# John-Jumper/Upside-MD

Hardware: AMD Instinct MI355X
Metric: MD steps/sec (force evals/sec) per 300-res protein (higher is better)
Workload: dtype f32; 1 GPU; syn300_10A: 300-res synthetic protein, full side-chain BP, 10 A pair list (BASELINE.json configs[2]); 4096 independent replicas per GPU, T=0.8, dt=0.009, Langevin thermostat every round; replicas_per_gpu=4096, n_atom=900, settle_steps=100

## Files before the change

upside-md_amd/csrc/engine.cpp:

```cpp
#include "engine.h"
#include "h5util.h"
#include <dlfcn.h>
#include <algorithm>
#include <cstdlib>
#include <set>
#include <functional>
#include <cmath>
#include <cstdio>
#include <cstring>

using namespace std;

void hip_check(hipError_t e, const char* what) {
    if (e != hipSuccess) throw string("HIP error in ") + what + ": " + hipGetErrorString(e);
}
void upk_check(int code, const char* what) {
    if (code == 0) return;
    if (code >= 9000) {
        const char* why = "";
        switch (code) {
            case 9003: why = ": more than 1024 rotamer nodes"; break;
            case 9004: case 9005: case 9006: why = ": the system does not fit the 160 KB of LDS this kernel stages it in"; break;
            case 9007: case 9008: why = ": side / mode / interaction type outside what the launcher implements"; break;
            case 9009: why = ": more than 65535 rows (row ids are 16 bits wide)"; break;
            case 9010: why = ": the graph's pair lists were allocated with another word width than its kernels read (upk_igraph_t::word16: 16-bit element "
                             "indices for every graph but the rotamer's, <= 65534 elements per side)"; break;
            case 9011: why = ": the hit-list refine exists for the side-chain graph (symmetric, 32-bit words) and for two-sided graphs with 16-bit words; "
                             "a symmetric radial graph walks its cached lists and has no hit lists"; break;
            default: break;
        }
        throw string("kernel launcher ") + what + " rejected its arguments (code " + to_string(code) + ")" + why;
    }
    throw string("HIP launch failure in ") + what + ": " + hipGetErrorString((hipError_t)code);
}

void DeviceCtx::flush() { upk_check(upk_fuse_flush(&L), "fuse_flush"); }
void DeviceCtx::begin(const std::string& fam) {
    if (!profile) return;
    flush();
    hipEvent_t a, b;
    hip_check(hipEventCreate(&a), "hipEventCreate"); hip_check(hipEventCreate(&b), "hipEventCreate");
    hip_check(hipEventRecord(a, stream), "hipEventRecord");
    families[fam].pending.emplace_back(a, b);
}
void DeviceCtx::end(const std::string& fam, double algorithmic_bytes, double pair_evaluations) {
    if (!profile) return;
    flush();
    auto& f = families[fam];
    hip_check(hipEventRecord(f.pending.back().second, stream), "hipEventRecord");
    f.launches += 1; f.bytes += algorithmic_bytes; f.pairs += pair_evaluations;
}
void DeviceCtx::flush_profile() {
    for (auto& kv : families) {
        for (auto& ev : kv.second.pending) {
            hip_check(hipEventSynchronize(ev.second), "hipEventSynchronize");
            float ms = 0.f;
            hip_check(hipEventElapsedTime(&ms, ev.first, ev.second), "hipEventElapsedTime");
            kv.second.ms += ms;
            (void)hipEventDestroy(ev.first); (void)hipEventDestroy(ev.second);
        }
        kv.second.pending.clear();
    }
}

int ScatterPlan::add_source(int n_term, int n_slot, int w, const vector<int>& targets) {
    if (finalized) throw string("scatter plan already finalized");
    if ((int)targets.size() != n_term * n_slot) throw string("scatter source: wrong target table size");
    if (width && width != w) throw string("scatter sources of one node must share a width");
    width = w;
    Source s; s.n_term = n_term; s.n_slot = n_slot; s.width = w; s.targets = targets; s.offset = arena_size;
    arena_size += (long)n_term * n_slot * w;
    sources.push_back(move(s));
    return (int)sources.size() - 1;
}
void ScatterPlan::finalize(int n_target, int n_system) {
    vector<int> count(n_target + 1, 0);
    for (auto& s : sources) for (int t : s.targets) if (t >= 0) { if (t >= n_target) throw string("scatter target out of range"); count[t + 1]++; }
    for (int t = 0; t < n_target; ++t) count[t + 1] += count[t];
    vector<int> fill(count.begin(), count.end() - 1), entry(count[n_target]);
    for (auto& s : sources)
        for (int i = 0; i < (int)s.targets.size(); ++i) {
            int t = s.targets[i];
            if (t >= 0) entry[fill[t]++] = (int)(s.offset + (long)i * s.width);
        }
    csr_start.upload(count); csr_entry.upload(entry);
    arena.alloc((size_t)n_system * (size_t)max(arena_size, 1L));
    finalized = true;
}

CoordNode::CoordNode(DeviceCtx* c, int n_elem_, int elem_width_)
    : DerivComputation(false), n_elem(n_elem_), elem_width(elem_width_), stride(ru(elem_width_)) {
    ctx = c;
    output.alloc((size_t)c->n_system * n_elem * stride);
    sens.alloc((size_t)c->n_system * n_elem * stride);
}
void CoordNode::gather_contributions() {
    if (scatter.sources.empty()) return;
    upk_check(upk_gather_contrib(&ctx->L, scatter.arena.p, scatter.arena_size, scatter.csr_start.p, scatter.csr_entry.p, coord(),
                                 scatter.width, 0), "gather_contrib");
}

namespace {
vector<int> identity_targets(int n) { vector<int> v(n); for (int i = 0; i < n; ++i) v[i] = i; return v; }

void fetch_dense(DeviceCtx* ctx, const CoordNode& n, const float* dev, vector<float>& stage, vector<float>& dst) {
    const size_t total = (size_t)ctx->n_system * n.n_elem * n.stride;
    stage.resize(total); dst.resize((size_t)ctx->n_system * n.n_elem * n.elem_width);
    if (!total) return;
    hip_check(hipMemcpyAsync(stage.data(), dev, total * sizeof(float), hipMemcpyDeviceToHost, ctx->stream), "D2H");
    hip_check(hipStreamSynchronize(ctx->stream), "hipStreamSynchronize");
    for (size_t e = 0; e < (size_t)ctx->n_system * n.n_elem; ++e)
        for (int d = 0; d < n.elem_width; ++d) dst[e * n.elem_width + d] = stage[e * n.stride + d];
}

void push_arg_derivs(DeviceCtx* ctx, const vector<CoordNode*>& args, const vector<int>& src, const vector<vector<float>>& din) {
    for (size_t a = 0; a < args.size(); ++a) {
        CoordNode& n = *args[a];
        const size_t per_sys = (size_t)n.n_elem * n.elem_width;
        for (int s = 0; s < ctx->n_system && per_sys; ++s)
            hip_check(hipMemcpyAsync(n.scatter.source_ptr(src[a]) + (size_t)s * n.scatter.arena_size, din[a].data() + s * per_sys,
                                     per_sys * sizeof(float), hipMemcpyHostToDevice, ctx->stream), "H2D");
    }
    hip_check(hipStreamSynchronize(ctx->stream), "hipStreamSynchronize");
}
}

HostPotentialNode::HostPotentialNode(DeviceCtx* c, const vector<CoordNode*>& args_) : PotentialNode(c), args(args_) {
    for (CoordNode* a : args) src_.push_back(a->scatter.add_source(a->n_elem, 1, a->elem_width, identity_targets(a->n_elem)));
    in_.resize(args.size()); din_.resize(args.size()); stage_.resize(args.size());
}
void HostPotentialNode::compute_value(ComputeMode) {
    for (size_t a = 0; a < args.size(); ++a) {
        fetch_dense(ctx, *args[a], args[a]->output.p, stage_[a], in_[a]);
        din_[a].assign(in_[a].size(), 0.f);
    }
    vector<const float*> in(args.size()); vector<float*> din(args.size());
    for (int s = 0; s < ctx->n_system; ++s) {
        for (size_t a = 0; a < args.size(); ++a) {
            const size_t off = (size_t)s * args[a]->n_elem * args[a]->elem_width;
            in[a] = in_[a].data() + off; din[a] = din_[a].data() + off;
        }
        potential[s] = host_potential(s, in, din);
    }
    hip_check(hipMemcpyAsync(potential_dev.p, potential.data(), ctx->n_system * sizeof(float), hipMemcpyHostToDevice, ctx->stream), "H2D");
    push_arg_derivs(ctx, args, src_, din_);
}

HostCoordNode::HostCoordNode(DeviceCtx* c, int n_elem_, int elem_width_, const vector<CoordNode*>& args_)
    : CoordNode(c, n_elem_, elem_width_), args(args_) {
    for (CoordNode* a : args) src_.push_back(a->scatter.add_source(a->n_elem, 1, a->elem_width, identity_targets(a->n_elem)));
    in_.resize(args.size()); din_.resize(args.size()); stage_.resize(args.size());
}
void HostCoordNode::compute_value(ComputeMode) {
    for (size_t a = 0; a < args.size(); ++a) fetch_dense(ctx, *args[a], args[a]->output.p, stage_[a], in_[a]);
    out_.assign((size_t)ctx->n_system * n_elem * stride, 0.f);
    vector<const float*> in(args.size()); vector<float> dense((size_t)n_elem * elem_width);
    for (int s = 0; s < ctx->n_system; ++s) {
        for (size_t a = 0; a < args.size(); ++a) in[a] = in_[a].data() + (size_t)s * args[a]->n_elem * args[a]->elem_width;
        host_value(s, in, dense.data());
        for (int e = 0; e < n_elem; ++e) for (int d = 0; d < elem_width; ++d) out_[((size_t)s * n_elem + e) * stride + d] = dense[(size_t)e * elem_width + d];
    }
    if (!out_.empty()) hip_check(hipMemcpyAsync(output.p, out_.data(), out_.size() * sizeof(float), hipMemcpyHostToDevice, ctx->stream), "H2D");
    hip_check(hipStreamSynchronize(ctx->stream), "hipStreamSynchronize");
}
void HostCoordNode::propagate_deriv() {
    vector<float> stage;
    fetch_dense(ctx, *this, sens.p, stage, dout_);
    vector<const float*> in(args.size()); vector<float*> din(args.size());
    for (size_t a = 0; a < args.size(); ++a) din_[a].assign(in_[a].size(), 0.f);
    for (int s = 0; s < ctx->n_system; ++s) {
        for (size_t a = 0; a < args.size(); ++a) {
            const size_t off = (size_t)s * args[a]->n_elem * args[a]->elem_width;
            in[a] = in_[a].data() + off; din[a] = din_[a].data() + off;
        }
        host_deriv(s, in, dout_.data() + (size_t)s * n_elem * elem_width, din);
    }
    push_arg_derivs(ctx, args, src_, din_);
}

NodeCreationMap& node_creation_map() {
    static NodeCreationMap m;
// ... 892 lines not shown
```

upside-md_amd/csrc/kernels_igraph.hip:

```cpp
#include "igraph_device.h"
#include <cstring>

using namespace up;

#define ST(L) ((hipStream_t)(L)->stream)
#define ROWS_PER_BLOCK 4
#define IG_BLOCK (ROWS_PER_BLOCK * UP_WAVE)
#ifndef UPK_LAUNCH_STATUS_DEFINED
#define UPK_LAUNCH_STATUS_DEFINED
static inline int launch_status() { return (int)hipGetLastError(); }
#endif
static inline unsigned rows_grid(int n_rows) { return n_rows > 0 ? (unsigned)((n_rows + ROWS_PER_BLOCK - 1) / ROWS_PER_BLOCK) : 1u; }

#define C_OUT(c, s)  ((c).out  + (size_t)(s) * (c).n_elem * (c).stride)
#define C_SENS(c, s) ((c).sens + (size_t)(s) * (c).n_elem * (c).stride)


__device__ __forceinline__ float quadspline(const upk_igraph_t& G, const float* __restrict__ p, const float* x1, const float* x2,
                                            float* d1, float* d2) {
    const int ka = G.n_knot_angular, k = G.n_knot;
    const float inv_dx = G.inv_dx, inv_dtheta = G.inv_dtheta;
    const f3 displace = mk3(x2[0] - x1[0], x2[1] - x1[1], x2[2] - x1[2]);
    const f3 rvec1 = mk3(x1[3], x1[4], x1[5]), rvec2 = mk3(x2[3], x2[4], x2[5]);
    const float dist2 = mag2(displace), inv_dist = rsqrt_(dist2);
// ... 113 lines not shown
    }
    __syncthreads();
    if (moved) {
        for (int e = threadIdx.x; e < n_tot; e += blockDim.x) {
            const bool side1 = e < G.n1;
            const int i = side1 ? e : e - G.n1;
            const upk_coord_t& node = side1 ? G.node1 : G.node2;
            const float* x = C_OUT(node, s) + (size_t)(side1 ? G.loc1[i] : G.loc2[i]) * node.stride;
            float4* c = (float4*)(side1 ? G.cache_pos1 + (size_t)s * G.n1 * 4 : G.cache_pos2 + (size_t)s * G.n2 * 4) + i;
            *c = make_float4(x[0], x[1], x[2], __int_as_float(side1 ? G.id1[i] : G.id2[i]));
        }
        if (G.mark_table) {
            uint4* m = (uint4*)(G.mark_table + (size_t)s * G.mark_stride);
            const int n16 = G.mark_stride / 16;
            for (int i = threadIdx.x; i < n16; i += blockDim.x) m[i] = make_uint4(0, 0, 0, 0);
        }
    }
    if (threadIdx.x == 0) {
        G.rebuild_flag[s] = moved;
        int* fl = UPK_FLAG_LIST(G);
        if (moved) fl[1 + atomicAdd(&fl[0], 1)] = s;
        if (s == 0) G.flagged[(size_t)(G.parity ^ 1) * G.flag_stride] = 0;
    }
}
__global__ void k_pairlist_check(upk_igraph_t G)  { d_pairlist_check(G, BX_REAL, nullptr); }
extern "C" int upk_pairlist_check(const upk_launch_t* L, const upk_igraph_t* G) {
    if (batch_add(L, BK_CHECK, 1, L->n_system, 0, G, sizeof(*G))) return 0;
    UPK_FLUSH(L);
    const int n_tot = G->symmetric ? G->n1 : G->n1 + G->n2;
    const int threads = plan_upkeep_block(L->n_system, upk_device_cu_count(), n_tot <= 256 ? 256 : (n_tot <= 512 ? 512 : 1024));
    hipLaunchKernelGGL(k_pairlist_check, dim3(1, L->n_system), dim3(threads), 0, ST(L), *G);
    return launch_status();
}

template <int IT>
__device__ __forceinline__ bool plb_id_ok(int id_row_side1, int id_other_side2) {
    if (IT == UPK_IT_ROTAMER) return ((unsigned)(id_row_side1 ^ id_other_side2)) > 15u;
    if (IT == UPK_IT_HBOND_COVERAGE || IT == UPK_IT_ENVIRONMENT || IT == UPK_IT_RADIAL || IT == UPK_IT_HBOND_SC_RADIAL) { const int d = id_row_side1 - id_other_side2; return (d > 2) | (d < -2); }
    return true;
}
__device__ __forceinline__ int plb_node_of(const upk_igraph_t& G, int id) {
    const int nr = (id >> 4) & 15;
    return (id >> 8) + ((-(int)(nr == 6) & G.mark_start6) | (-(int)(nr == 3) & G.mark_start3));
}
template <bool STAGED, int IT>
__device__ __forceinline__ void d_pairlist_build(const upk_igraph_t& G, int blocks1, int rows_per_wg, const BX B, float* plb_lds) {
        float4* oth = (float4*)plb_lds;
    constexpr bool SYM = IT == UPK_IT_ROTAMER || IT == UPK_IT_RADIAL;
    constexpr bool UPPER = IT == UPK_IT_ROTAMER;
    const int* fl = UPK_FLAG_LIST(G);
    const int n_flagged = fl[0];
    const int lane = threadIdx.x & 63, wave = __builtin_amdgcn_readfirstlane(threadIdx.x >> 6), n_wave = blockDim.x >> 6;
    const bool side1 = (int)B.bx < blocks1;
    const int rb = side1 ? B.bx : B.bx - blocks1;
    const int n_my = side1 ? G.n1 : G.n2, n_other = side1 ? G.n2 : G.n1;
    const int n_pad = (n_other + 63) & ~63;
    const int cap = side1 ? G.cap1 : G.cap2;
    const float cut2 = G.cache_cutoff * G.cache_cutoff;
    for (int fi = B.by; fi < n_flagged; fi += B.gy) {
        const int s = fl[1 + fi];
        const float4* src = (const float4*)((side1 ? G.cache_pos2 : G.cache_pos1) + (size_t)s * n_other * 4);
        const float4* mine = (const float4*)((side1 ? G.cache_pos1 : G.cache_pos2) + (size_t)s * n_my * 4);
        if (STAGED) {
            __syncthreads();
            for (int j = threadIdx.x; j < n_pad; j += blockDim.x) oth[j] = j < n_other ? src[j] : make_float4(1e18f, 1e18f, 1e18f, 0.f);
            __syncthreads();
        }
        float4 x_next = make_float4(0.f, 0.f, 0.f, 0.f);
        { const int i0 = rb * rows_per_wg + wave; if (wave < rows_per_wg && i0 < n_my) x_next = mine[i0]; }
        for (int r = wave; r < rows_per_wg; r += n_wave) {
            const int i = rb * rows_per_wg + r;
            if (i >= n_my) break;
            const float4 x = x_next;
            { const int in = i + n_wave; if (r + n_wave < rows_per_wg && in < n_my) x_next = mine[in]; }
            const int my_id = __float_as_int(x.w);
            typedef typename list_word<IT>::type W;
            W* nbr = (side1 ? (W*)G.nbr1 + (size_t)s * G.n1 * G.cap1 : (W*)G.nbr2 + (size_t)s * G.n2 * G.cap2) + (size_t)i * cap;
            int count = 0;
            const int my_node = SYM ? plb_node_of(G, my_id) : 0;
            for (int j0 = UPPER ? ((i + 1) & ~63) : 0; j0 < n_pad; j0 += 64) {
                const int j = j0 + lane;
                float4 y;
                if (STAGED) y = oth[j];
                else y = j < n_other ? src[j] : make_float4(1e18f, 1e18f, 1e18f, 0.f);
                const float d2 = dist2_exact(x.x, x.y, x.z, y.x, y.y, y.z);
                const int oid = __float_as_int(y.w);
                bool hit = (d2 < cut2) & (side1 ? plb_id_ok<IT>(my_id, oid) : plb_id_ok<IT>(oid, my_id));
                if (UPPER) hit = hit & (j > i);
                else if (SYM) hit = hit & (j != i);
                const unsigned long long b = __ballot(hit);
                if (!b) continue;
                const int pos = count + __popcll(b & ((1ull << lane) - 1ull));
                if (hit & (pos < cap)) nbr[pos] = (W)j;
                count += __popcll(b);
                if (SYM && G.mark_table) {
                    const bool up = hit & (j > i);
                    const int key = up ? plb_node_of(G, oid) : -1;
                    const int key_prev = __builtin_amdgcn_update_dpp(-1, key, 0x138 , 0xf, 0xf, false);
                    if (up & (key_prev != key)) {
                        unsigned char* mt = G.mark_table + (size_t)s * G.mark_stride;
                        mt[my_node * G.mark_ld + key] = 1; mt[key * G.mark_ld + my_node] = 1;
                    }
                }
            }
            if (lane == 0) {
                (side1 ? G.cnt1 + (size_t)s * G.n1 : G.cnt2 + (size_t)s * G.n2)[i] = count < cap ? count : cap;
                if (count > cap) *G.error_flag = 1;
            }
        }
    }
}
template <bool STAGED, int IT>
__global__ void __launch_bounds__(1024) k_pairlist_build(upk_igraph_t G, int blocks1, int rows_per_wg)  {
    extern __shared__ __attribute__((aligned(16))) float lds_dyn_[];
    d_pairlist_build<STAGED, IT>(G, blocks1, rows_per_wg, BX_REAL, lds_dyn_);
}
template <int IT>
static void plb_launch(const upk_launch_t* L, const upk_igraph_t* G, dim3 grid, size_t lds, bool staged, int blocks1) {
    const int rows = plan_list_build_rows(L->n_system, upk_device_cu_count());
    if (staged) hipLaunchKernelGGL((k_pairlist_build<true, IT>), grid, dim3(plan_upkeep_block(L->n_system, upk_device_cu_count(), 1024)), lds, ST(L), *G, blocks1, rows);
    else hipLaunchKernelGGL((k_pairlist_build<false, IT>), grid, dim3(1024), 0, ST(L), *G, blocks1, rows);
}
extern "C" int upk_pairlist_build(const upk_launch_t* L, const upk_igraph_t* G) { return upk_pairlist_build_sides(L, G, 3); }
extern "C" int upk_pairlist_build_sides(const upk_launch_t* L, const upk_igraph_t* G, int sides) {
    if (!list_words_match(G)) return 9010;
    const int rows = plan_list_build_rows(L->n_system, upk_device_cu_count());
    const int blocks1 = (sides & 1) ? (G->n1 + rows - 1) / rows : 0;
    const int blocks2 = (G->symmetric || !(sides & 2)) ? 0 : (G->n2 + rows - 1) / rows;
    if (blocks1 + blocks2 == 0) return 0;
    const int n_max = G->n1 > G->n2 ? G->n1 : G->n2;
    const size_t lds = (size_t)((n_max + 63) & ~63) * 16;
    const dim3 grid(blocks1 + blocks2, UPK_FLAG_GRID(L->n_system));
    const bool staged = plan_list_build_staged(plan_switches(), lds);
    if (staged) {
        const int bk = G->itype == UPK_IT_ROTAMER ? BK_BUILD_ROT : G->itype == UPK_IT_HBOND_COVERAGE ? BK_BUILD_COV : G->itype == UPK_IT_ENVIRONMENT ? BK_BUILD_ENV
                     : G->itype == UPK_IT_PROTEIN_HBOND ? BK_BUILD_HB : 0;
        if (bk && batch_add(L, bk, (int)grid.x, (int)grid.y, lds, G, sizeof(*G), nullptr, 0, blocks1, rows)) return 0;
    }
    UPK_FLUSH(L);
    switch (G->itype) {
        case UPK_IT_ROTAMER: plb_launch<UPK_IT_ROTAMER>(L, G, grid, lds, staged, blocks1); break;
        case UPK_IT_HBOND_COVERAGE: plb_launch<UPK_IT_HBOND_COVERAGE>(L, G, grid, lds, staged, blocks1); break;
        case UPK_IT_ENVIRONMENT: plb_launch<UPK_IT_ENVIRONMENT>(L, G, grid, lds, staged, blocks1); break;
        case UPK_IT_RADIAL: plb_launch<UPK_IT_RADIAL>(L, G, grid, lds, staged, blocks1); break;
        case UPK_IT_HBOND_SC_RADIAL: plb_launch<UPK_IT_HBOND_SC_RADIAL>(L, G, grid, lds, staged, blocks1); break;
        default: plb_launch<UPK_IT_PROTEIN_HBOND>(L, G, grid, lds, staged, blocks1); break;
    }
    return launch_status();
}

#ifndef PLR_BLOCK
#define PLR_BLOCK 256
#endif
#ifndef PLR_DEPTH
#define PLR_DEPTH 2
#endif
static_assert(PLR_ROWS <= 64 * (PLR_BLOCK / 64), "a wavefront of the refine keeps the positions and list lengths of its rows one per lane: at most 64 rows per wavefront");
typedef float plr_v2 __attribute__((ext_vector_type(2)));
__device__ __forceinline__ plr_v2 dist2_exact2(plr_v2 ax, plr_v2 ay, plr_v2 az, plr_v2 bx, plr_v2 by, plr_v2 bz) {
#pragma clang fp contract(off)
    const plr_v2 dx = ax - bx, dy = ay - by, dz = az - bz;
    const plr_v2 xx = dx * dx, yy = dy * dy, zz = dz * dz;
    const plr_v2 s = xx + yy;
    return s + zz;
}
template <bool SYM, typename W>
__device__ __forceinline__ void d_pairlist_refine(const upk_igraph_t& G, int side, int rows_per_wg, const BX B, float* plr_lds) {
        float4* oth = (float4*)plr_lds;
    const int s = B.by;
    const int lane = threadIdx.x & 63, wave = __builtin_amdgcn_readfirstlane(threadIdx.x >> 6), n_wave = blockDim.x >> 6;
    const bool rows1 = side == 1;
    const int n_rows = rows1 ? G.n1 : G.n2, n_other = rows1 ? G.n2 : G.n1;
    const int cap = rows1 ? G.cap1 : G.cap2;
    const float4* src = (const float4*)((rows1 ? G.cur_pos2 : G.cur_pos1) + (size_t)s * n_other * 4);
    const float4* mine = (const float4*)((rows1 ? G.cur_pos1 : G.cur_pos2) + (size_t)s * n_rows * 4);
    for (int j = threadIdx.x; j <= n_other; j += blockDim.x) oth[j] = j < n_other ? src[j] : make_float4(1e18f, 1e18f, 1e18f, 0.f);
    __syncthreads();
    const int dead = n_other;
    const W* nbr_base = (const W*)(rows1 ? G.nbr1 : G.nbr2) + (size_t)s * n_rows * cap;
    const int* cnt_arr = (rows1 ? G.cnt1 : G.cnt2) + (size_t)s * n_rows;
    W* hit_base = (W*)(rows1 ? G.hit1 : G.hit2) + (size_t)s * n_rows * cap;
    int* hcnt = (rows1 ? G.hcnt1 : G.hcnt2) + (size_t)s * n_rows;
    int* hlo = (SYM && G.hlo1) ? G.hlo1 + (size_t)s * n_rows : nullptr;
    const float cut2 = G.cutoff * G.cutoff;
    const int jmask = G.nbr_j_bits ? (1 << G.nbr_j_bits) - 1 : 0x7fffffff;
    const int per_wave = (rows_per_wg + n_wave - 1) / n_wave;
    const int r0 = B.bx * rows_per_wg + wave * per_wave;
    int r1 = r0 + per_wave; { const int wg_end = (B.bx + 1) * rows_per_wg; if (r1 > wg_end) r1 = wg_end; if (r1 > n_rows) r1 = n_rows; }
    if (r0 >= r1) return;
    const bool have = r0 + lane < r1;
    const float4 my_x = have ? mine[r0 + lane] : make_float4(0.f, 0.f, 0.f, 0.f);
    const int my_cnt = have ? cnt_arr[r0 + lane] : 0;
    int my_n = 0, my_lo = 0;
    auto bcast = [&](float v, int l) { return __int_as_float(__builtin_amdgcn_readlane(__float_as_int(v), l)); };
    auto fetch_pair = [&](int ra, int& a, int& b) {
        a = dead; b = dead;
        if (ra < r1) {
            const int la = ra - r0;
            const int cA = __builtin_amdgcn_readlane(my_cnt, la & 63), cB = ra + 1 < r1 ? __builtin_amdgcn_readlane(my_cnt, (la + 1) & 63) : 0;
            if (lane < cA) a = nbr_base[(size_t)ra * cap + lane];
            if (lane < cB) b = nbr_base[(size_t)(ra + 1) * cap + lane];
        }
    };
    int qA[PLR_DEPTH], qB[PLR_DEPTH];
#pragma unroll
    for (int d = 0; d < PLR_DEPTH; ++d) fetch_pair(r0 + 2 * d, qA[d], qB[d]);
    for (int ra = r0; ra < r1; ra += 2) {
        const int la = ra - r0, lb = la + 1;
        const bool hasB = ra + 1 < r1;
        const int cntA = __builtin_amdgcn_readlane(my_cnt, la), cntB = hasB ? __builtin_amdgcn_readlane(my_cnt, lb & 63) : 0;
        int wA = qA[0], wB = qB[0];
#pragma unroll
        for (int d = 0; d + 1 < PLR_DEPTH; ++d) { qA[d] = qA[d + 1]; qB[d] = qB[d + 1]; }
        fetch_pair(ra + 2 * PLR_DEPTH, qA[PLR_DEPTH - 1], qB[PLR_DEPTH - 1]);
        plr_v2 xx, xy, xz;
        xx.x = bcast(my_x.x, la); xy.x = bcast(my_x.y, la); xz.x = bcast(my_x.z, la);
        xx.y = bcast(my_x.x, lb & 63); xy.y = bcast(my_x.y, lb & 63); xz.y = bcast(my_x.z, lb & 63);
        const W* nbrA = nbr_base + (size_t)ra * cap; const W* nbrB = nbrA + cap;
        W* outA = hit_base + (size_t)ra * cap; W* outB = outA + cap;
        int na = 0, nb = 0, loa = 0, lob = 0;
        const int cmax = cntA > cntB ? cntA : cntB;
        for (int k0 = 0; k0 < cmax; k0 += 64) {
            const int k = k0 + lane;
            if (k0) { wA = k < cntA ? nbrA[k] : dead; wB = k < cntB ? nbrB[k] : dead; }
            const int jA = wA & jmask, jB = wB & jmask;
            const float4 yA = oth[jA], yB = oth[jB];
            plr_v2 yx, yy, yz; yx.x = yA.x; yx.y = yB.x; yy.x = yA.y; yy.y = yB.y; yz.x = yA.z; yz.y = yB.z;
            const plr_v2 d2 = dist2_exact2(xx, xy, xz, yx, yy, yz);
            const bool hitA = d2.x < cut2, hitB = d2.y < cut2;
            const unsigned long long mA = __builtin_amdgcn_ballot_w64(hitA), mB = __builtin_amdgcn_ballot_w64(hitB);
            const unsigned long long below = (1ull << lane) - 1ull;
            if (hitA) outA[na + __popcll(mA & below)] = (W)wA;
            if (hitB) outB[nb + __popcll(mB & below)] = (W)wB;
            na += __popcll(mA); nb += __popcll(mB);
            if (SYM) { loa += __popcll(__builtin_amdgcn_ballot_w64(hitA && jA < ra)); lob += __popcll(__builtin_amdgcn_ballot_w64(hitB && jB < ra + 1)); }
        }
        if (lane == la) { my_n = na; my_lo = loa; }
        if (hasB && lane == lb) { my_n = nb; my_lo = lob; }
    }
    if (have) { hcnt[r0 + lane] = my_n; if (SYM && hlo) hlo[r0 + lane] = my_lo; }
}
template <bool SYM, typename W>
__global__ void __launch_bounds__(PLR_BLOCK) k_pairlist_refine(upk_igraph_t G, int side, int rows_per_wg)  {
    extern __shared__ __attribute__((aligned(16))) float lds_dyn_[];
    d_pairlist_refine<SYM, W>(G, side, rows_per_wg, BX_REAL, lds_dyn_);
}
__device__ __forceinline__ void d_pairlist_refine_short(const upk_igraph_t& G, int side, const BX B, float* lds_unused) {
    const int s = B.by, row = B.bx * blockDim.x + threadIdx.x;
    const bool rows1 = side == 1;
    const int n_rows = rows1 ? G.n1 : G.n2, n_other = rows1 ? G.n2 : G.n1;
    if (row >= n_rows) return;
    const int cap = rows1 ? G.cap1 : G.cap2;
    const float4* src = (const float4*)((rows1 ? G.cur_pos2 : G.cur_pos1) + (size_t)s * n_other * 4);
    const float4 x = ((const float4*)((rows1 ? G.cur_pos1 : G.cur_pos2) + (size_t)s * n_rows * 4))[row];
    typedef list_word<UPK_IT_PROTEIN_HBOND>::type W;
    const W* nbr = (const W*)(rows1 ? G.nbr1 : G.nbr2) + ((size_t)s * n_rows + row) * cap;
    W* hit = (W*)(rows1 ? G.hit1 : G.hit2) + ((size_t)s * n_rows + row) * cap;
    const int cnt = ((rows1 ? G.cnt1 : G.cnt2) + (size_t)s * n_rows)[row];
    const float cut2 = G.cutoff * G.cutoff;
    const int jmask = G.nbr_j_bits ? (1 << G.nbr_j_bits) - 1 : 0x7fffffff;
    int n = 0;
    for (int k0 = 0; k0 < cnt; k0 += 4) {
        int w[4]; float4 y[4];
#pragma unroll
        for (int u = 0; u < 4; ++u) w[u] = nbr[k0 + u < cnt ? k0 + u : k0];
#pragma unroll
        for (int u = 0; u < 4; ++u) y[u] = src[w[u] & jmask];
#pragma unroll
        for (int u = 0; u < 4; ++u)
            if (k0 + u < cnt && dist2_exact(x.x, x.y, x.z, y[u].x, y[u].y, y[u].z) < cut2) hit[n++] = (W)w[u];
    }
    ((rows1 ? G.hcnt1 : G.hcnt2) + (size_t)s * n_rows)[row] = n;
}
__global__ void __launch_bounds__(256) k_pairlist_refine_short(upk_igraph_t G, int side)  { d_pairlist_refine_short(G, side, BX_REAL, nullptr); }
extern "C" int upk_pairlist_refine(const upk_launch_t* L, const upk_igraph_t* G, int side) {
    const bool rows1 = side == 1;
    const int n_rows = rows1 ? G->n1 : G->n2, n_other = rows1 ? G->n2 : G->n1;
    if (n_rows < 1) return 0;
    if (G->itype == UPK_IT_PROTEIN_HBOND && !G->symmetric) {
        if (batch_add(L, BK_REFINE_SHORT, (n_rows + 1023) / 1024, L->n_system, 0, G, sizeof(*G), nullptr, 0, side)) return 0;
        UPK_FLUSH(L);
        hipLaunchKernelGGL(k_pairlist_refine_short, dim3((n_rows + 255) / 256, L->n_system), dim3(256), 0, ST(L), *G, side);
        return launch_status();
    }
    if (!list_words_match(G)) return 9010;
    if ((G->symmetric != 0) == (G->word16 != 0)) return 9011;
    const size_t lds = (size_t)((n_other > 0 ? n_other : 0) + 1) * 16;
    if (lds > PLAN_LIST_LDS) return 9006;
    const int rows_per_wg = plan_refine_rows(L->n_system, upk_device_cu_count(), n_rows);
    {
        const int rows_b = rows_per_wg * 4;
        if (batch_add(L, G->symmetric ? BK_REFINE_SYM : BK_REFINE, (n_rows + rows_b - 1) / rows_b, L->n_system, lds, G, sizeof(*G), nullptr, 0, side, rows_b)) return 0;
    }
    UPK_FLUSH(L);
    const dim3 grid((n_rows + rows_per_wg - 1) / rows_per_wg, L->n_system);
    if (G->symmetric) hipLaunchKernelGGL((k_pairlist_refine<true, int>), grid, dim3(PLR_BLOCK), lds, ST(L), *G, side, rows_per_wg);
    else hipLaunchKernelGGL((k_pairlist_refine<false, unsigned short>), grid, dim3(PLR_BLOCK), lds, ST(L), *G, side, rows_per_wg);

    return launch_status();
}

#define PLO_BINS 1024
template <typename KeyFn>
__device__ __forceinline__ void order_rows(unsigned short* __restrict__ ord, int n_rows, KeyFn key, int* hist, int* scratch) {
    hist[threadIdx.x] = 0;
    __syncthreads();
    for (int r = threadIdx.x; r < n_rows; r += blockDim.x) atomicAdd(&hist[PLO_BINS - 1 - key(r)], 1);
    __syncthreads();
    const int lane = threadIdx.x & 63, wave = threadIdx.x >> 6;
    const int v = hist[threadIdx.x];
    int incl = v;
#pragma unroll
    for (int off = 1; off < 64; off <<= 1) { const int t = __shfl_up(incl, off, UP_WAVE); if (lane >= off) incl += t; }
    if (lane == 63) scratch[wave] = incl;
    __syncthreads();
    if (threadIdx.x == 0) { int acc = 0; for (int w = 0; w < (int)(blockDim.x >> 6); ++w) { const int t = scratch[w]; scratch[w] = acc; acc += t; } }
    __syncthreads();
    hist[threadIdx.x] = scratch[wave] + incl - v;
    __syncthreads();
    for (int r = threadIdx.x; r < n_rows; r += blockDim.x) ord[atomicAdd(&hist[PLO_BINS - 1 - key(r)], 1)] = (unsigned short)r;
    __syncthreads();
}
__device__ __forceinline__ void d_pairlist_order(const upk_igraph_t& G, int side, const BX B, float* lds_unused) {
    __shared__ int hist[PLO_BINS], scratch[16];
    const int s = B.bx;
    const bool rows1 = side == 1;
    const int n_rows = rows1 ? G.n1 : G.n2;
    const int* hcnt = (rows1 ? G.hcnt1 : G.hcnt2) + (size_t)s * n_rows;
    order_rows((rows1 ? G.ord1 : G.ord2) + (size_t)s * n_rows, n_rows,
               [&](int r) { const int c = hcnt[r]; return c < PLO_BINS ? c : PLO_BINS - 1; }, hist, scratch);
    if (G.symmetric && G.hlo1) {
        const int* hlo = G.hlo1 + (size_t)s * n_rows;
        order_rows(G.ord1u + (size_t)s * n_rows, n_rows,
                   [&](int r) { const int c = hcnt[r] - hlo[r]; return c < PLO_BINS ? c : PLO_BINS - 1; }, hist, scratch);
    }
}
__global__ void __launch_bounds__(PLO_BINS) k_pairlist_order(upk_igraph_t G, int side)  { d_pairlist_order(G, side, BX_REAL, nullptr); }
extern "C" int upk_pairlist_order(const upk_launch_t* L, const upk_igraph_t* G, int side) {
    const int n_rows = side == 1 ? G->n1 : G->n2;
    if (n_rows < 1) return 0;
    if (n_rows > 65535) return 9009;
    if (batch_add(L, BK_ORDER, L->n_system, 1, 0, G, sizeof(*G), nullptr, 0, side)) return 0;
    UPK_FLUSH(L);
    hipLaunchKernelGGL(k_pairlist_order, dim3(L->n_system), dim3(PLO_BINS), 0, ST(L), *G, side);
    return launch_status();
}

__global__ void k_igraph_rowsum(upk_igraph_t G, int side, float* __restrict__ out, long out_sys_stride, int out_stride, int out_comp,
                                int out_row0, float* __restrict__ own_grad) {
    const int s = blockIdx.y;
    const int lane = threadIdx.x & 63;
    const int n_rows = side == 1 ? G.n1 : G.n2;
    const float cut2 = G.cutoff * G.cutoff;
    for (int row = blockIdx.x * ROWS_PER_BLOCK + (threadIdx.x >> 6); row < n_rows; row += gridDim.x * ROWS_PER_BLOCK) {
        const int cap = side == 1 ? G.cap1 : G.cap2;
        const int* lists = side == 1 ? G.nbr1 : G.nbr2;
        const size_t row_at = ((size_t)s * n_rows + row) * cap;
        const int cnt = (side == 1 ? G.cnt1 + (size_t)s * G.n1 : G.cnt2 + (size_t)s * G.n2)[row];
        float xr[8];
        if (side == 1) load_elem(xr, G.node1, s, G.loc1[row], G.dim1); else load_elem(xr, G.node2, s, G.loc2[row], G.dim2);
        const int tr = side == 1 ? G.type1[row] : G.type2[row];
        float acc = 0.f, og[8];
#pragma unroll
        for (int c = 0; c < 8; ++c) og[c] = 0.f;
        for (int k = lane; k < cnt; k += 64) {
            const int j = list_word_at(lists, row_at + k, G.word16);
            float xo[8], d1[8], d2[8];
#pragma unroll
            for (int c = 0; c < 8; ++c) { d1[c] = 0.f; d2[c] = 0.f; }
            if (side == 1) load_elem(xo, G.node2, s, G.loc2[j], G.dim2); else load_elem(xo, G.node1, s, G.loc1[j], G.dim1);
            if (!(dist2_exact(xr[0], xr[1], xr[2], xo[0], xo[1], xo[2]) < cut2)) continue;
            const int t1 = side == 1 ? tr : G.type1[j], t2 = side == 1 ? G.type2[j] : tr;
            const float* p = G.param + (size_t)(t1 * G.n_type2 + t2) * G.n_param;
            acc += side == 1 ? pair_eval(G, p, xr, xo, d1, d2) : pair_eval(G, p, xo, xr, d1, d2);
#pragma unroll
            for (int c = 0; c < 8; ++c) og[c] += side == 1 ? d1[c] : d2[c];
        }
        acc = wave_sum(acc);
        if (lane == 0) out[(size_t)s * out_sys_stride + (size_t)(out_row0 + row) * out_stride + out_comp] = acc;
        if (own_grad) {
#pragma unroll
            for (int c = 0; c < 8; ++c) og[c] = wave_sum(og[c]);
            if (lane == 0) {
                float* o = own_grad + ((size_t)s * n_rows + row) * 8;
#pragma unroll
                for (int c = 0; c < 8; ++c) o[c] = og[c];
            }
        }
    }
}
extern "C" int upk_igraph_rowsum(const upk_launch_t* L, const upk_igraph_t* G, int side, float* out, long out_sys_stride,
                                 int out_stride, int out_comp, int out_row0, float* own_grad) {
    UPK_FLUSH(L);
    const int n_rows = side == 1 ? G->n1 : G->n2;
    hipLaunchKernelGGL(k_igraph_rowsum, dim3(rows_grid(n_rows), L->n_system), dim3(IG_BLOCK), 0, ST(L), *G, side,
                       out, out_sys_stride, out_stride, out_comp, out_row0, own_grad);
    return launch_status();
}

__global__ void k_igraph_grad(upk_igraph_t G, int side, int sens_mode, const float* __restrict__ sens1, const float* __restrict__ sens2,
                              long sens_sys_stride, int sens_stride) {
    const int s = blockIdx.y;
    const int lane = threadIdx.x & 63;
    const int n_rows = side == 1 ? G.n1 : G.n2;
    const int dim_row = side == 1 ? G.dim1 : G.dim2;
    const float cut2 = G.cutoff * G.cutoff;
    const float* S1 = sens1 ? sens1 + (size_t)s * sens_sys_stride : nullptr;
    const float* S2 = sens2 ? sens2 + (size_t)s * sens_sys_stride : nullptr;
    for (int row = blockIdx.x * ROWS_PER_BLOCK + (threadIdx.x >> 6); row < n_rows; row += gridDim.x * ROWS_PER_BLOCK) {
        const int cap = side == 1 ? G.cap1 : G.cap2;
        const int* lists = side == 1 ? G.nbr1 : G.nbr2;
        const size_t row_at = ((size_t)s * n_rows + row) * cap;
        const int cnt = (side == 1 ? G.cnt1 + (size_t)s * G.n1 : G.cnt2 + (size_t)s * G.n2)[row];
        float xr[8];
        if (side == 1) load_elem(xr, G.node1, s, G.loc1[row], G.dim1); else load_elem(xr, G.node2, s, G.loc2[row], G.dim2);
        const int tr = side == 1 ? G.type1[row] : G.type2[row];
        float srow = 0.f;
        if (sens_mode == 1 && side == 1) srow = S1[(size_t)row * sens_stride];
        if (sens_mode == 2 && side == 2) srow = S2[(size_t)row * sens_stride];
        if (sens_mode == 3) srow = side == 1 ? S1[(size_t)row * sens_stride] : S2[(size_t)row * sens_stride];
        float acc[8];
#pragma unroll
        for (int c = 0; c < 8; ++c) acc[c] = 0.f;
        for (int k = lane; k < cnt; k += 64) {
            const int j = list_word_at(lists, row_at + k, G.word16);
            float xo[8], d1[8], d2[8];
#pragma unroll
            for (int c = 0; c < 8; ++c) { d1[c] = 0.f; d2[c] = 0.f; }
            if (side == 1) load_elem(xo, G.node2, s, G.loc2[j], G.dim2); else load_elem(xo, G.node1, s, G.loc1[j], G.dim1);
            if (!(dist2_exact(xr[0], xr[1], xr[2], xo[0], xo[1], xo[2]) < cut2)) continue;
            const int t1 = side == 1 ? tr : G.type1[j], t2 = side == 1 ? G.type2[j] : tr;
            const float* p = G.param + (size_t)(t1 * G.n_type2 + t2) * G.n_param;
            if (side == 1) pair_eval(G, p, xr, xo, d1, d2); else pair_eval(G, p, xo, xr, d1, d2);
            float ps;
            if (sens_mode == 0) ps = 1.f;
            else if (sens_mode == 1) ps = side == 1 ? srow : S1[(size_t)j * sens_stride];
            else if (sens_mode == 2) ps = side == 2 ? srow : S2[(size_t)j * sens_stride];
            else ps = srow + (side == 1 ? S2[(size_t)j * sens_stride] : S1[(size_t)j * sens_stride]);
// ... 163 lines not shown
```

upside-md_amd/csrc/launch_plan.h:

```cpp
#pragma once
#include "env_switch.h"
#include <climits>
#include <cstddef>

#ifndef PG_LANES
#define PG_LANES 8
#endif
#ifndef P2_LANES
#define P2_LANES 4
#endif
#define PG_WALK_LDS_WORDS(n_rows) ((n_rows) + ((n_rows) + 1) / 2)
#ifndef PLR_ROWS
#define PLR_ROWS 256
#endif
#define BP_BLOCK 1024
#ifndef BP_NODE_STRIDE
#define BP_NODE_STRIDE 6
#endif
#define BP_NODE_ARRAYS 2
#ifndef BPL_THREADS
#define BPL_THREADS 512
#endif
#define BPC_BLOCK 512
enum { N_CLASS = 5 };

constexpr size_t PLAN_CU_LDS = 160 * 1024;
constexpr size_t PLAN_PAIR_LDS = 158 * 1024;
constexpr size_t PLAN_BP_CLUSTER_LDS = 156 * 1024;
constexpr size_t PLAN_BP_BASE_LDS = 155 * 1024;
constexpr size_t PLAN_BP_LAYOUT_LDS = 40 * 1024;
constexpr size_t PLAN_LIST_LDS = 150 * 1024;

struct PlanSwitches {
    int BATCH = INT_MIN;
    int GRAPH = -1;
    int ASYNC_PREPARE = 1, FUSE = 1, FUSE_BARRIERS = 0, FUSE_THREADS = 0;
    float SKIN_SCALE = 0.f;
    int NBR_CAP = 512, ADJ_CAP = 256;
    float SLOT_FACTOR = 96.f;
    int SLOT_SPLIT = 0, IG_WGS = 256, IG_POLY = 1, ROT_POLY = 1, IG_UNSTAGED = 0, ROT_UNSTAGED = 0, PLB_UNSTAGED = 0, PAIR2 = 1;
    int ROT_SORT_BEADS = 1, ROTAMER_ATOMIC = 0, MAX_ROTAMER_NODES = 1024;
    int BP_CLUSTER = -1;
    int BP_CLUSTER_TEST_ABORT = 0, BP_COMPACT = 1;
    int BP_LAYOUT = -1;
    int BP_ENERGY_TABLE = 0, BP_LDS_MSG_KB = 160, NODE_PROB_IN_SOLVE = 1;
    int BACKBONE_LIST = 1;
    float BACKBONE_SKIN = 3.f;
    int BACKBONE_LIST_CAP = 128;
};
inline const PlanSwitches& plan_switches() {
    static const PlanSwitches sw = [] {
        PlanSwitches s;
        s.BATCH = env_int("UPSIDE_HIP_BATCH", s.BATCH); s.GRAPH = env_int("UPSIDE_HIP_GRAPH", s.GRAPH);
        s.ASYNC_PREPARE = env_int("UPSIDE_HIP_ASYNC_PREPARE", s.ASYNC_PREPARE); s.FUSE = env_int("UPSIDE_HIP_FUSE", s.FUSE);
        s.FUSE_BARRIERS = env_int("UPSIDE_HIP_FUSE_BARRIERS", s.FUSE_BARRIERS); s.FUSE_THREADS = env_int("UPSIDE_HIP_FUSE_THREADS", s.FUSE_THREADS);
        s.NBR_CAP = env_int("UPSIDE_HIP_NBR_CAP", s.NBR_CAP); s.ADJ_CAP = env_int("UPSIDE_HIP_ADJ_CAP", s.ADJ_CAP);
        s.SLOT_SPLIT = env_int("UPSIDE_HIP_SLOT_SPLIT", s.SLOT_SPLIT); s.IG_WGS = env_int("UPSIDE_HIP_IG_WGS", s.IG_WGS);
        s.IG_POLY = env_int("UPSIDE_HIP_IG_POLY", s.IG_POLY); s.ROT_POLY = env_int("UPSIDE_HIP_ROT_POLY", s.ROT_POLY);
        s.IG_UNSTAGED = env_int("UPSIDE_HIP_IG_UNSTAGED", s.IG_UNSTAGED); s.ROT_UNSTAGED = env_int("UPSIDE_HIP_ROT_UNSTAGED", s.ROT_UNSTAGED);
        s.PLB_UNSTAGED = env_int("UPSIDE_HIP_PLB_UNSTAGED", s.PLB_UNSTAGED); s.PAIR2 = env_int("UPSIDE_HIP_PAIR2", s.PAIR2);
        s.ROT_SORT_BEADS = env_int("UPSIDE_HIP_ROT_SORT_BEADS", s.ROT_SORT_BEADS);
        s.ROTAMER_ATOMIC = env_int("UPSIDE_HIP_ROTAMER_ATOMIC", s.ROTAMER_ATOMIC);
        s.MAX_ROTAMER_NODES = env_int("UPSIDE_HIP_MAX_ROTAMER_NODES", s.MAX_ROTAMER_NODES);
        s.BP_CLUSTER = env_int("UPSIDE_HIP_BP_CLUSTER", s.BP_CLUSTER);
        s.BP_CLUSTER_TEST_ABORT = env_int("UPSIDE_HIP_BP_CLUSTER_TEST_ABORT", s.BP_CLUSTER_TEST_ABORT);
        s.BP_COMPACT = env_int("UPSIDE_HIP_BP_COMPACT", s.BP_COMPACT); s.BP_LAYOUT = env_int("UPSIDE_HIP_BP_LAYOUT", s.BP_LAYOUT);
        s.BP_ENERGY_TABLE = env_int("UPSIDE_HIP_BP_ENERGY_TABLE", s.BP_ENERGY_TABLE);
        s.BP_LDS_MSG_KB = env_int("UPSIDE_HIP_BP_LDS_MSG_KB", s.BP_LDS_MSG_KB);
        s.NODE_PROB_IN_SOLVE = env_int("UPSIDE_HIP_NODE_PROB_IN_SOLVE", s.NODE_PROB_IN_SOLVE);
        s.BACKBONE_LIST = env_int("UPSIDE_HIP_BACKBONE_LIST", s.BACKBONE_LIST);
        s.BACKBONE_LIST_CAP = env_int("UPSIDE_HIP_BACKBONE_LIST_CAP", s.BACKBONE_LIST_CAP);
        s.SKIN_SCALE = env_float("UPSIDE_HIP_SKIN_SCALE", s.SKIN_SCALE); s.SLOT_FACTOR = env_float("UPSIDE_HIP_SLOT_FACTOR", s.SLOT_FACTOR);
        s.BACKBONE_SKIN = env_float("UPSIDE_HIP_BACKBONE_SKIN", s.BACKBONE_SKIN);
        return s;
    }();
    return sw;
}

inline bool plan_merged_launches(const PlanSwitches& sw, int S, int n_atom) {
    if (sw.BATCH != INT_MIN) return sw.BATCH != 0;
    return S <= 16 || ((long)S * n_atom <= 24000 && S <= 160);
}
inline bool plan_graph_replay(const PlanSwitches& sw, bool merged, bool fuse_trace) {
    return fuse_trace ? false : (sw.GRAPH >= 0 ? sw.GRAPH != 0 : merged);
}
inline int plan_fuse_lanes(const PlanSwitches& sw, int S, bool heavy) {
    const int forced = (sw.FUSE_THREADS % 64 || sw.FUSE_THREADS > 1024) ? 0 : sw.FUSE_THREADS;
    const int t = forced ? forced : (S >= 2048 ? 256 : (S >= 256 ? 512 : 1024));
    return heavy && t > 512 ? 512 : t;
}
inline bool plan_heavy_op_alone(int S, int n) { return S >= 256 || n > 64; }

struct BackboneList { bool on; int cap; float skin; };
inline BackboneList plan_backbone_list(const PlanSwitches& sw, int n_residue) {
    return {n_residue > 128 && sw.BACKBONE_LIST != 0, n_residue < sw.BACKBONE_LIST_CAP ? n_residue : sw.BACKBONE_LIST_CAP, sw.BACKBONE_SKIN};
}

inline float plan_skin_scale(const PlanSwitches& sw, int S, bool side_chain_graph) {
    if (sw.SKIN_SCALE > 0.f) return sw.SKIN_SCALE;
    if (S <= 16) return 1.5f;
    return (S <= 256 || side_chain_graph) ? 0.5f : 0.75f;
}
inline bool plan_gacc(bool symmetric, int S) { return !symmetric && S < 256; }

struct PairGeometry { int wgs_per_system, lanes; };
inline PairGeometry plan_pair_geometry(const PlanSwitches& sw, int S, int n_rows, int lanes_per_row, int rows_per_full_wg) {
    const int target = sw.IG_WGS < 1 ? 256 : sw.IG_WGS;
    int bps = (target + S - 1) / S;
    const int max_bps = (n_rows + rows_per_full_wg - 1) / rows_per_full_wg;
    if (bps > max_bps) bps = max_bps;
    if (bps < 1) bps = 1;
    const int rows_per_wg = (n_rows + bps - 1) / bps;
    const int t = ((rows_per_wg * lanes_per_row + 63) / 64) * 64;
    return {bps, t < 256 ? 256 : (t > 1024 ? 1024 : t)};
}
inline PairGeometry plan_pair_geometry(const PlanSwitches& sw, int S, int n_rows, bool packed) {
    return packed ? plan_pair_geometry(sw, S, n_rows, P2_LANES, 256) : plan_pair_geometry(sw, S, n_rows, PG_LANES, 128);
}

struct PairShape { bool coverage, has_poly; int n1, n2, cap1, cap2, n_type1, n_type2, n_param, n_poly; };
enum PlanTable { PLAN_TABLE_NONE = 0, PLAN_TABLE_COEF = 1, PLAN_TABLE_POLY = 2 };
struct PairTable { PlanTable table; int tab_floats; size_t lds_bytes; };
inline PairTable plan_pair_table(const PlanSwitches& sw, const PairShape& g, size_t extra) {
    const int n_max = g.n1 > g.n2 ? g.n1 : g.n2;
    for (int poly = 1; poly >= 0; --poly) {
        if (poly && (!sw.IG_POLY || !g.has_poly)) continue;
        const int tab_floats = g.n_type1 * g.n_type2 * (poly ? g.n_poly : g.n_param);
        const size_t bytes = ((size_t)((tab_floats + 3) & ~3) + (size_t)(g.n1 + g.n2) * 8 + PG_WALK_LDS_WORDS(n_max) + 4) * sizeof(float);
        if (bytes <= PLAN_PAIR_LDS && !sw.IG_UNSTAGED && n_max < 65536 && g.cap1 < 65536 && g.cap2 < 65536 && bytes + extra <= PLAN_PAIR_LDS)
            return {poly ? PLAN_TABLE_POLY : PLAN_TABLE_COEF, tab_floats, bytes};
    }
    return {PLAN_TABLE_NONE, 0, 0};
}
struct PairPass { PlanTable table; bool packed; int tab_floats; size_t lds_bytes; };
inline PairPass plan_pair_forward(const PlanSwitches& sw, const PairShape& g, int side, int mode) {
    const PairTable t = plan_pair_table(sw, g, 0);
    const bool packed = t.table && g.coverage && mode == 0 && side != 3 && sw.PAIR2 && t.lds_bytes + 64 <= PLAN_PAIR_LDS;
    return {t.table, packed, t.tab_floats, t.lds_bytes + (packed ? 64 : 0)};
}
inline PairPass plan_pair_backward(const PlanSwitches& sw, const PairShape& g, int row_side, int d_other) {
    const int n_other = row_side == 1 ? g.n2 : g.n1;
    const size_t acc_bytes = 8 + (size_t)n_other * d_other * sizeof(unsigned long long);
    const PairTable t = plan_pair_table(sw, g, acc_bytes);
    if (t.table && g.coverage && sw.PAIR2) {
        const size_t extra = 64 + (size_t)g.n1 * sizeof(float);
        const PairTable t2 = plan_pair_table(sw, g, acc_bytes + extra);
        if (t2.table) return {t2.table, true, t2.tab_floats, t2.lds_bytes + acc_bytes + extra};
    }
    return {t.table, false, t.tab_floats, t.lds_bytes + acc_bytes};
}
inline bool plan_passes_staged(const PlanSwitches& sw, const PairShape& g, int row_side) {
    if (row_side != 1 && row_side != 2) return false;
    const int n_other = row_side == 1 ? g.n2 : g.n1;
    return plan_pair_table(sw, g, 0).table && plan_pair_table(sw, g, 8 + (size_t)n_other * 8 * sizeof(unsigned long long)).table;
}
struct TableSlices { int rows, n_slice; };
inline TableSlices plan_pd_table_slices(int n_rows, int n_param) {
    const size_t row_bytes = (size_t)(n_param > 0 ? n_param : 1) * sizeof(unsigned long long);
    const int fit = (int)(PLAN_PAIR_LDS / row_bytes);
    if (fit < 1 || n_rows < 1) return {0, 0};
    const int n_slice = (n_rows + fit - 1) / fit;
    return {(n_rows + n_slice - 1) / n_slice, n_slice};
}

inline int plan_upkeep_block(int S, int n_cu, int large) { return S >= 2 * n_cu ? 256 : large; }
inline int plan_list_build_rows(int S, int n_cu) { return S >= n_cu ? 128 : 64; }
// ... 87 lines not shown
```

Baseline: 221,400 system-steps/s.

## Refine pair lists with sub-wavefront lane groups per row and deeper prefetch

Restructures the pair-list refine kernel. Previously each whole wavefront walked two rows at a time with 64 lanes each. Now each wavefront is split into groups of 16 lanes, with one row per group, so four rows are handled concurrently. Each group uses its slice of the ballot to compact hits, and a double-buffered RowSet prefetches the next rows' neighbor words, counts and positions up to 128 entries ahead. The aim is to stop wasting lanes when neighbor lists are much shorter than 64 entries and to hide global-load latency. It also adds a guard that rejects 16-bit word graphs that pack extra bits beside the index, because the new code reads such a word as the index directly.

```diff
diff --git a/upside-md_amd/csrc/engine.cpp b/upside-md_amd/csrc/engine.cpp
--- a/upside-md_amd/csrc/engine.cpp
+++ b/upside-md_amd/csrc/engine.cpp
@@ -27,6 +27,8 @@
                              "indices for every graph but the rotamer's, <= 65534 elements per side)"; break;
             case 9011: why = ": the hit-list refine exists for the side-chain graph (symmetric, 32-bit words) and for two-sided graphs with 16-bit words; "
                              "a symmetric radial graph walks its cached lists and has no hit lists"; break;
+            case 9012: why = ": a graph with 16-bit list words packs bits beside the partner's index (upk_igraph_t::nbr_j_bits): the refine reads such a "
+                             "word as the index itself"; break;
             default: break;
         }
         throw string("kernel launcher ") + what + " rejected its arguments (code " + to_string(code) + ")" + why;
diff --git a/upside-md_amd/csrc/kernels_igraph.hip b/upside-md_amd/csrc/kernels_igraph.hip
--- a/upside-md_amd/csrc/kernels_igraph.hip
+++ b/upside-md_amd/csrc/kernels_igraph.hip
@@ -289,93 +289,85 @@
 #ifndef PLR_BLOCK
 #define PLR_BLOCK 256
 #endif
-#ifndef PLR_DEPTH
-#define PLR_DEPTH 2
-#endif
-static_assert(PLR_ROWS <= 64 * (PLR_BLOCK / 64), "a wavefront of the refine keeps the positions and list lengths of its rows one per lane: at most 64 rows per wavefront");
-typedef float plr_v2 __attribute__((ext_vector_type(2)));
-__device__ __forceinline__ plr_v2 dist2_exact2(plr_v2 ax, plr_v2 ay, plr_v2 az, plr_v2 bx, plr_v2 by, plr_v2 bz) {
-#pragma clang fp contract(off)
-    const plr_v2 dx = ax - bx, dy = ay - by, dz = az - bz;
-    const plr_v2 xx = dx * dx, yy = dy * dy, zz = dz * dz;
-    const plr_v2 s = xx + yy;
-    return s + zz;
-}
-template <bool SYM, typename W>
+template <bool SYM, typename W, int LPR = SYM ? PLR_LPR_SYM : PLR_LPR_W16>
 __device__ __forceinline__ void d_pairlist_refine(const upk_igraph_t& G, int side, int rows_per_wg, const BX B, float* plr_lds) {
-        float4* oth = (float4*)plr_lds;
+    static_assert(LPR == 16 || LPR == 32, "a group's bit field of the ballot is taken with 32-bit operations");
+    static_assert(PLR_AHEAD % LPR == 0 && PLR_AHEAD >= LPR, "whole trips in flight");
+    constexpr int NG = 64 / LPR, U = PLR_AHEAD / LPR;
+    float4* oth = (float4*)plr_lds;
     const int s = B.by;
     const int lane = threadIdx.x & 63, wave = __builtin_amdgcn_readfirstlane(threadIdx.x >> 6), n_wave = blockDim.x >> 6;
     const bool rows1 = side == 1;
     const int n_rows = rows1 ? G.n1 : G.n2, n_other = rows1 ? G.n2 : G.n1;
     const int cap = rows1 ? G.cap1 : G.cap2;
     const float4* src = (const float4*)((rows1 ? G.cur_pos2 : G.cur_pos1) + (size_t)s * n_other * 4);
-    const float4* mine = (const float4*)((rows1 ? G.cur_pos1 : G.cur_pos2) + (size_t)s * n_rows * 4);
     for (int j = threadIdx.x; j <= n_other; j += blockDim.x) oth[j] = j < n_other ? src[j] : make_float4(1e18f, 1e18f, 1e18f, 0.f);
     __syncthreads();
     const int dead = n_other;
-    const W* nbr_base = (const W*)(rows1 ? G.nbr1 : G.nbr2) + (size_t)s * n_rows * cap;
-    const int* cnt_arr = (rows1 ? G.cnt1 : G.cnt2) + (size_t)s * n_rows;
-    W* hit_base = (W*)(rows1 ? G.hit1 : G.hit2) + (size_t)s * n_rows * cap;
-    int* hcnt = (rows1 ? G.hcnt1 : G.hcnt2) + (size_t)s * n_rows;
-    int* hlo = (SYM && G.hlo1) ? G.hlo1 + (size_t)s * n_rows : nullptr;
     const float cut2 = G.cutoff * G.cutoff;
     const int jmask = G.nbr_j_bits ? (1 << G.nbr_j_bits) - 1 : 0x7fffffff;
     const int per_wave = (rows_per_wg + n_wave - 1) / n_wave;
     const int r0 = B.bx * rows_per_wg + wave * per_wave;
     int r1 = r0 + per_wave; { const int wg_end = (B.bx + 1) * rows_per_wg; if (r1 > wg_end) r1 = wg_end; if (r1 > n_rows) r1 = n_rows; }
     if (r0 >= r1) return;
-    const bool have = r0 + lane < r1;
-    const float4 my_x = have ? mine[r0 + lane] : make_float4(0.f, 0.f, 0.f, 0.f);
-    const int my_cnt = have ? cnt_arr[r0 + lane] : 0;
-    int my_n = 0, my_lo = 0;
-    auto bcast = [&](float v, int l) { return __int_as_float(__builtin_amdgcn_readlane(__float_as_int(v), l)); };
-    auto fetch_pair = [&](int ra, int& a, int& b) {
-        a = dead; b = dead;
-        if (ra < r1) {
-            const int la = ra - r0;
-            const int cA = __builtin_amdgcn_readlane(my_cnt, la & 63), cB = ra + 1 < r1 ? __builtin_amdgcn_readlane(my_cnt, (la + 1) & 63) : 0;
-            if (lane < cA) a = nbr_base[(size_t)ra * cap + lane];
-            if (lane < cB) b = nbr_base[(size_t)(ra + 1) * cap + lane];
-        }
+    const int n_run = r1 - r0;
+    const size_t run0 = (size_t)s * n_rows + r0;
+    const float4* mine = (const float4*)(rows1 ? G.cur_pos1 : G.cur_pos2) + run0;
+    const int* cnt_arr = (rows1 ? G.cnt1 : G.cnt2) + run0;
+    const char* nbr_run = (const char*)((const W*)(rows1 ? G.nbr1 : G.nbr2) + run0 * cap);
+    char* hit_run = (char*)((W*)(rows1 ? G.hit1 : G.hit2) + run0 * cap);
+    int* hcnt = (rows1 ? G.hcnt1 : G.hcnt2) + run0;
+    int* hlo = (SYM && G.hlo1) ? G.hlo1 + run0 : nullptr;
+    const unsigned row_bytes = (unsigned)cap * (unsigned)sizeof(W);
+    const int grp = lane / LPR, sub = lane % LPR;
+    const unsigned gshift = grp * LPR, gmask = LPR == 32 ? 0xffffffffu : (1u << LPR) - 1u, below = (1u << sub) - 1u;
+    auto ld_cnt = [&](int b) { const int lr = b + grp, c = cnt_arr[lr < n_run ? lr : n_run - 1]; return lr < n_run ? c : 0; };
+    struct RowSet { int cnt; float4 x; int cmax; int q[U]; };
+    auto fetch = [&](int b, RowSet& S) {
+        const int lr = b + grp;
+        S.x = mine[lr < n_run ? lr : n_run - 1];
+        S.cmax = 0;
+#pragma unroll
+        for (int g = 0; g < NG; ++g) { const int c = __builtin_amdgcn_readlane(S.cnt, g * LPR); S.cmax = c > S.cmax ? c : S.cmax; }
+        const W* mine_words = (const W*)(nbr_run + ((unsigned)lr * row_bytes + (unsigned)sub * (unsigned)sizeof(W)));
+#pragma unroll
+        for (int u = 0; u < U; ++u) S.q[u] = (u * LPR < S.cmax && u * LPR + sub < S.cnt) ? (int)mine_words[u * LPR] : dead;
     };
-    int qA[PLR_DEPTH], qB[PLR_DEPTH];
-#pragma unroll
-    for (int d = 0; d < PLR_DEPTH; ++d) fetch_pair(r0 + 2 * d, qA[d], qB[d]);
-    for (int ra = r0; ra < r1; ra += 2) {
-        const int la = ra - r0, lb = la + 1;
-        const bool hasB = ra + 1 < r1;
-        const int cntA = __builtin_amdgcn_readlane(my_cnt, la), cntB = hasB ? __builtin_amdgcn_readlane(my_cnt, lb & 63) : 0;
-        int wA = qA[0], wB = qB[0];
-#pragma unroll
-        for (int d = 0; d + 1 < PLR_DEPTH; ++d) { qA[d] = qA[d + 1]; qB[d] = qB[d + 1]; }
-        fetch_pair(ra + 2 * PLR_DEPTH, qA[PLR_DEPTH - 1], qB[PLR_DEPTH - 1]);
-        plr_v2 xx, xy, xz;
-        xx.x = bcast(my_x.x, la); xy.x = bcast(my_x.y, la); xz.x = bcast(my_x.z, la);
-        xx.y = bcast(my_x.x, lb & 63); xy.y = bcast(my_x.y, lb & 63); xz.y = bcast(my_x.z, lb & 63);
-        const W* nbrA = nbr_base + (size_t)ra * cap; const W* nbrB = nbrA + cap;
-        W* outA = hit_base + (size_t)ra * cap; W* outB = outA + cap;
-        int na = 0, nb = 0, loa = 0, lob = 0;
-        const int cmax = cntA > cntB ? cntA : cntB;
-        for (int k0 = 0; k0 < cmax; k0 += 64) {
-            const int k = k0 + lane;
-            if (k0) { wA = k < cntA ? nbrA[k] : dead; wB = k < cntB ? nbrB[k] : dead; }
-            const int jA = wA & jmask, jB = wB & jmask;
-            const float4 yA = oth[jA], yB = oth[jB];
-            plr_v2 yx, yy, yz; yx.x = yA.x; yx.y = yB.x; yy.x = yA.y; yy.y = yB.y; yz.x = yA.z; yz.y = yB.z;
-            const plr_v2 d2 = dist2_exact2(xx, xy, xz, yx, yy, yz);
-            const bool hitA = d2.x < cut2, hitB = d2.y < cut2;
-            const unsigned long long mA = __builtin_amdgcn_ballot_w64(hitA), mB = __builtin_amdgcn_ballot_w64(hitB);
-            const unsigned long long below = (1ull << lane) - 1ull;
-            if (hitA) outA[na + __popcll(mA & below)] = (W)wA;
-            if (hitB) outB[nb + __popcll(mB & below)] = (W)wB;
-            na += __popcll(mA); nb += __popcll(mB);
-            if (SYM) { loa += __popcll(__builtin_amdgcn_ballot_w64(hitA && jA < ra)); lob += __popcll(__builtin_amdgcn_ballot_w64(hitB && jB < ra + 1)); }
-        }
-        if (lane == la) { my_n = na; my_lo = loa; }
-        if (hasB && lane == lb) { my_n = nb; my_lo = lob; }
-    }
-    if (have) { hcnt[r0 + lane] = my_n; if (SYM && hlo) hlo[r0 + lane] = my_lo; }
+    auto refine_set = [&](int b, const RowSet& S) {
+        const int lr = b + grp, row = r0 + lr;
+        const unsigned out = (unsigned)lr * row_bytes;
+        int n = 0, lo = 0;
+        auto test = [&](int w) {
+            const int j = sizeof(W) == 2 ? w : w & jmask;
+            const float4 y = oth[j];
+            const bool h = dist2_exact(S.x.x, S.x.y, S.x.z, y.x, y.y, y.z) < cut2;
+            const unsigned long long m = __builtin_amdgcn_ballot_w64(h);
+            const unsigned gb = (unsigned)(m >> gshift) & gmask;
+            if (h) *(W*)(hit_run + (out + (unsigned)(n + __popc(gb & below)) * (unsigned)sizeof(W))) = (W)w;
+            n += __popc(gb);
+            if (SYM) lo += __popc((unsigned)((__builtin_amdgcn_ballot_w64(j < row) & m) >> gshift) & gmask);
+        };
+#pragma unroll
+        for (int u = 0; u < U; ++u) { if (u * LPR >= S.cmax) break; test(S.q[u]); }
+        for (int k = U * LPR + sub; k - sub < S.cmax; k += LPR)
+            test(k < S.cnt ? (int)*(const W*)(nbr_run + (out + (unsigned)k * (unsigned)sizeof(W))) : dead);
+        if (sub == 0 && lr < n_run) { hcnt[lr] = n; if (SYM && hlo) hlo[lr] = lo; }
+    };
+    RowSet A, Bs;
+    A.cnt = ld_cnt(0); Bs.cnt = ld_cnt(NG);
+    fetch(0, A);
+    for (int b = 0;;) {
+        int after = ld_cnt(b + 2 * NG);
+        fetch(b + NG, Bs);
+        refine_set(b, A);
+        A.cnt = after; b += NG;
+        if (b >= n_run) break;
+        after = ld_cnt(b + 2 * NG);
+        fetch(b + NG, A);
+        refine_set(b, Bs);
+        Bs.cnt = after; b += NG;
+        if (b >= n_run) break;
+    }
 }
 template <bool SYM, typename W>
 __global__ void __launch_bounds__(PLR_BLOCK) k_pairlist_refine(upk_igraph_t G, int side, int rows_per_wg)  {
@@ -421,6 +413,7 @@
         return launch_status();
     }
     if (!list_words_match(G)) return 9010;
+    if (G->word16 && G->nbr_j_bits) return 9012;
     if ((G->symmetric != 0) == (G->word16 != 0)) return 9011;
     const size_t lds = (size_t)((n_other > 0 ? n_other : 0) + 1) * 16;
     if (lds > PLAN_LIST_LDS) return 9006;
diff --git a/upside-md_amd/csrc/launch_plan.h b/upside-md_amd/csrc/launch_plan.h
--- a/upside-md_amd/csrc/launch_plan.h
+++ b/upside-md_amd/csrc/launch_plan.h
@@ -12,6 +12,15 @@
 #define PG_WALK_LDS_WORDS(n_rows) ((n_rows) + ((n_rows) + 1) / 2)
 #ifndef PLR_ROWS
 #define PLR_ROWS 256
+#endif
+#ifndef PLR_LPR_SYM
+#define PLR_LPR_SYM 16
+#endif
+#ifndef PLR_LPR_W16
+#define PLR_LPR_W16 16
+#endif
+#ifndef PLR_AHEAD
+#define PLR_AHEAD 128
 #endif
 #define BP_BLOCK 1024
 #ifndef BP_NODE_STRIDE
```

Result: faster. 223,900 system-steps/s (median of 6 runs) (+1.2%).
